# DeepGraphLearning/ULTRA

Measured on AMD Instinct MI355X. Metric: triples scored/sec (all-tail ranking) on FB15k237, higher is better.
Workload: dtype f32

## Files before the change

ultra_amd/csrc/dense_order_layer.hip:

```cpp
#include <hip/hip_runtime.h>

#include <cstdint>
#include <cstdlib>
#include <string>

#ifndef ULTRA_DOL_ASM
#define ULTRA_DOL_ASM 0
#endif
#if ULTRA_DOL_ASM
#include ULTRA_DOL_ASM_HEADER
#endif
#include "plan.hpp"
#include "torch_math.hpp"

#pragma clang fp contract(off)

namespace ultra {

using f32x4 = float __attribute__((ext_vector_type(4)));

enum { DOL_LN = 1, DOL_RELU = 2, DOL_RESIDUAL = 4 };

struct DenseOrderParams {
    const uint4 *a_ex;
    const float *rel, *x, *bnd;
    const long long *bnd_rows;
    const float *weight, *bias, *ln_w, *ln_b;
    float *out;
    long long rel_so, rel_sr, x_so, x_sr, bnd_so, bnd_sr, out_so, out_sr;
    int n_out, n_in, n_rel, n_jc, n_rt16, has_bnd, flags;
    float eps;
};

constexpr int DOL_ROW_STRIDE = 68;

__device__ __forceinline__ float byte_of(uint32_t w, int q) { return (float)((w >> (8 * q)) & 0xffu); }

#ifdef ULTRA_DOL_VGPR_CAP
#define ULTRA_DOL_ATTR __attribute__((amdgpu_waves_per_eu(4, 4)))
#else
#define ULTRA_DOL_ATTR
#endif
template <int TILES, bool LEAN, int SUBS = 1>
__device__ __forceinline__ void dense_order_layer_impl(const DenseOrderParams &p) {
    __shared__ __attribute__((aligned(16))) float x_lds_all[SUBS * TILES * 16 * DOL_ROW_STRIDE];
    __shared__ __attribute__((aligned(16))) float agg_lds_all[SUBS * TILES * 16 * DOL_ROW_STRIDE];
    __shared__ float ln_mom_all[SUBS][TILES * 16][8][2];
    __shared__ float ln_stat_all[SUBS][TILES * 16][2];
    const int sub = SUBS > 1 ? __builtin_amdgcn_readfirstlane((int)threadIdx.x >> 8) : 0;
    float *x_lds = x_lds_all + sub * (TILES * 16 * DOL_ROW_STRIDE), *agg_lds = agg_lds_all + sub * (TILES * 16 * DOL_ROW_STRIDE);
    float(&ln_mom)[TILES * 16][8][2] = ln_mom_all[sub];
    float(&ln_stat)[TILES * 16][2] = ln_stat_all[sub];
    const int tid = threadIdx.x & 255, lane = tid & 63;
    const int wave = __builtin_amdgcn_readfirstlane(tid >> 6);
    const int i16 = lane & 15, kk = lane >> 4;
    const int n_wt = (p.n_rt16 + TILES * SUBS - 1) / (TILES * SUBS);
    const int rt_raw = (blockIdx.x % n_wt) * SUBS + sub, outer = blockIdx.x / n_wt;
    const bool quartet_live = rt_raw * TILES < p.n_rt16;
    const int rt = quartet_live ? rt_raw : (p.n_rt16 - 1) / TILES;
    const float *xo = p.x + (long long)outer * p.x_so;
    const int row0 = rt * 16 * TILES;
    const int c0 = 16 * wave;
    const bool tile1 = TILES > 1 && TILES * rt + 1 < p.n_rt16;

    const uint4 *ap[TILES];
#pragma unroll
    for (int t = 0; t < TILES; ++t) ap[t] = p.a_ex + (size_t)min(TILES * rt + t, p.n_rt16 - 1) * p.n_jc * 64;
    const char *xbase = reinterpret_cast<const char *>(xo);
    const uint32_t x_row_bytes = (uint32_t)p.x_sr * 4u;
    const uint32_t lane_bytes = (uint32_t)(c0 + i16) * 4u;
#if !ULTRA_DOL_ASM
    uint32_t voff[16], voff_last[LEAN ? 1 : 16];
#pragma unroll
    for (int q = 0; q < 16; ++q) {
        voff[q] = (uint32_t)q * x_row_bytes + lane_bytes;
        if (!LEAN) voff_last[q] = (uint32_t)min(16 * (p.n_jc - 1) + q, p.n_in - 1) * x_row_bytes + lane_bytes;
    }
    const uint32_t off_max = (uint32_t)(p.n_in - 1 - 16 * (p.n_jc - 1)) * x_row_bytes + lane_bytes;
    struct Stage {
        uint4 a[TILES];
        float x[16];
    };
    const auto fetch = [&](const int jc, Stage &st) {
        const bool last = jc >= p.n_jc - 1;
        const int jcc = last ? p.n_jc - 1 : jc;
#pragma unroll
        for (int t = 0; t < TILES; ++t) st.a[t] = ap[t][(size_t)jcc * 64 + lane];
        if (LEAN) {
            const char *sbase = xbase + (uint32_t)jcc * 16u * x_row_bytes;
            const uint32_t cap = last ? off_max : 0xffffffffu;
#pragma unroll
            for (int q = 0; q < 16; ++q) st.x[q] = *reinterpret_cast<const float *>(sbase + min(voff[q], cap));
        } else {
            const char *sbase = xbase + (last ? 0u : (uint32_t)jcc * 16u * x_row_bytes);
#pragma unroll
            for (int q = 0; q < 16; ++q) st.x[q] = *reinterpret_cast<const float *>(sbase + (last ? voff_last[q] : voff[q]));
        }
    };
    Stage st0, st1, st2;
    fetch(0, st0);
    fetch(1, st1);
    fetch(2, st2);
#endif
    const float relv = kk < p.n_rel ? p.rel[(long long)outer * p.rel_so + (long long)kk * p.rel_sr + c0 + i16] : 0.f;

    float4 xtile[TILES];
    float wfrag[32];
    const int f0 = 16 * wave + 4 * kk;
    float biasv[4], lnw[4], lnb[4];
    float bndv[TILES][4];
    const auto fetch_late_operands = [&]() {
#pragma unroll
        for (int t = 0; t < TILES; ++t) {
            const int row = min(row0 + 16 * t + (tid >> 4), p.n_out - 1);
            xtile[t] = *reinterpret_cast<const float4 *>(xo + (long long)row * p.x_sr + 4 * (tid & 15));
        }
#pragma unroll
        for (int s = 0; s < 32; ++s) wfrag[s] = p.weight[(16 * wave + i16) * 128 + 4 * s + kk];
#pragma unroll
        for (int r = 0; r < 4; ++r) {
            biasv[r] = p.bias ? p.bias[f0 + r] : 0.f;
            lnw[r] = (p.flags & DOL_LN) ? p.ln_w[f0 + r] : 1.f;
            lnb[r] = (p.flags & DOL_LN) ? p.ln_b[f0 + r] : 0.f;
        }
#pragma unroll
        for (int t = 0; t < TILES; ++t)
#pragma unroll
            for (int r = 0; r < 4; ++r) bndv[t][r] = 0.f;
        if (p.has_bnd) {
            const long long bnd_row = p.bnd_rows ? p.bnd_rows[outer] : -1;
#pragma unroll
            for (int t = 0; t < TILES; ++t)
#pragma unroll
                for (int r = 0; r < 4; ++r) {
                    const int row = row0 + 16 * t + 4 * kk + r;
                    if (row < p.n_out && (bnd_row < 0 || bnd_row == row))
                        bndv[t][r] = p.bnd[(long long)outer * p.bnd_so + (long long)row * p.bnd_sr + c0 + i16];
                }
        }
    };
    if (!LEAN) fetch_late_operands();

    f32x4 acc[TILES];
#pragma unroll
    for (int t = 0; t < TILES; ++t)
#pragma unroll
        for (int r = 0; r < 4; ++r) acc[t][r] = 0.f;
#if ULTRA_DOL_ASM
    static_assert(TILES == 1, "the assembly chain of the measurement build walks one tile");
    dense_order_chain_asm(acc[0], p.n_jc, p.n_in, (uint32_t)lane * 16u, ap[0], xbase, lane_bytes, x_row_bytes, relv, (uint32_t)tid * 128u);
#else
    const auto chain = [&](const Stage &cur, const int jc) {
        const uint32_t m = jc < p.n_jc ? 0xffffffffu : 0u;
        uint32_t aw[TILES][4];
#pragma unroll
        for (int t = 0; t < TILES; ++t) {
            aw[t][0] = cur.a[t].x & m, aw[t][1] = cur.a[t].y & m, aw[t][2] = cur.a[t].z & m, aw[t][3] = cur.a[t].w & m;
        }
#pragma unroll
        for (int q = 0; q < 16; ++q) {
            const float b = relv * cur.x[q];
#pragma unroll
            for (int t = 0; t < TILES; ++t)
                acc[t] = __builtin_amdgcn_mfma_f32_16x16x4f32(byte_of(aw[t][q >> 2], q & 3), b, acc[t], 0, 0, 0);
        }
    };
    for (int jc = 0; jc < p.n_jc; jc += 3) {
        chain(st0, jc);
        fetch(jc + 3, st0);
        chain(st1, jc + 1);
        fetch(jc + 4, st1);
        chain(st2, jc + 2);
        fetch(jc + 5, st2);
    }
#endif

    if (LEAN) fetch_late_operands();

#pragma unroll
    for (int t = 0; t < TILES; ++t) {
#pragma unroll
        for (int r = 0; r < 4; ++r) {
            float v = acc[t][r];
            if (p.has_bnd) v += bndv[t][r];
            agg_lds[(16 * t + 4 * kk + r) * DOL_ROW_STRIDE + c0 + i16] = v;
        }
        *reinterpret_cast<float4 *>(x_lds + (16 * t + (tid >> 4)) * DOL_ROW_STRIDE + 4 * (tid & 15)) = xtile[t];
    }
    __syncthreads();

    f32x4 d[TILES];
#pragma unroll
    for (int t = 0; t < TILES; ++t) {
#pragma unroll
        for (int r = 0; r < 4; ++r) d[t][r] = 0.f;
#pragma unroll
        for (int s = 0; s < 16; ++s)
            d[t] = __builtin_amdgcn_mfma_f32_16x16x4f32(wfrag[s], x_lds[(16 * t + i16) * DOL_ROW_STRIDE + 4 * s + kk], d[t], 0, 0, 0);
#pragma unroll
        for (int s = 0; s < 16; ++s)
            d[t] = __builtin_amdgcn_mfma_f32_16x16x4f32(wfrag[16 + s], agg_lds[(16 * t + i16) * DOL_ROW_STRIDE + 4 * s + kk], d[t], 0, 0, 0);
    }
    float y[TILES][4];
#pragma unroll
    for (int t = 0; t < TILES; ++t)
#pragma unroll
        for (int r = 0; r < 4; ++r) y[t][r] = d[t][r] + biasv[r];
    if (p.flags & DOL_LN) {
        __syncthreads();
#pragma unroll
        for (int t = 0; t < TILES; ++t)
#pragma unroll
            for (int r = 0; r < 4; ++r) agg_lds[(16 * t + i16) * DOL_ROW_STRIDE + f0 + r] = y[t][r];
        __syncthreads();
        if (tid < 128 * TILES) {
            const int row = tid >> 3, i = tid & 7;
            float xv[8];
#pragma unroll
            for (int j = 0; j < 8; ++j) xv[j] = agg_lds[row * DOL_ROW_STRIDE + 8 * j + i];
            const Moments w = welford8(xv);
            ln_mom[row][i][0] = w.m1;
            ln_mom[row][i][1] = w.m2;
        }
        __syncthreads();
        if (tid < 16 * TILES) {
            Moments all[8];
#pragma unroll
            for (int i = 0; i < 8; ++i) all[i] = Moments{ln_mom[tid][i][0], ln_mom[tid][i][1]};
            float mean, rstd;
            merge8(all, p.eps, mean, rstd);
            ln_stat[tid][0] = mean;
            ln_stat[tid][1] = rstd;
        }
        __syncthreads();
#pragma unroll
        for (int t = 0; t < TILES; ++t) {
            const float mean = ln_stat[16 * t + i16][0], rstd = ln_stat[16 * t + i16][1];
#pragma unroll
            for (int r = 0; r < 4; ++r) y[t][r] = ln_apply(y[t][r], mean, rstd, lnw[r], lnb[r]);
        }
    }
#pragma unroll
    for (int t = 0; t < TILES; ++t) {
        if (p.flags & DOL_RELU) {
#pragma unroll
            for (int r = 0; r < 4; ++r) y[t][r] = fmaxf(y[t][r], 0.f);
        }
        if (p.flags & DOL_RESIDUAL) {
#pragma unroll
            for (int r = 0; r < 4; ++r) y[t][r] += x_lds[(16 * t + i16) * DOL_ROW_STRIDE + f0 + r];
        }
        const int row = row0 + 16 * t + i16;
        if (row < p.n_out && (t == 0 || tile1) && quartet_live)
            *reinterpret_cast<float4 *>(p.out + (long long)outer * p.out_so + (long long)row * p.out_sr + f0) =
                make_float4(y[t][0], y[t][1], y[t][2], y[t][3]);
    }
}

template <int TILES>
__global__ void __launch_bounds__(256) ULTRA_DOL_ATTR dense_order_layer_kernel(const DenseOrderParams p) {
    dense_order_layer_impl<TILES, false>(p);
}

__global__ void __launch_bounds__(256) __attribute__((amdgpu_waves_per_eu(4, 4))) dense_order_layer_lean_kernel(const DenseOrderParams p) {
    dense_order_layer_impl<1, true>(p);
}

__global__ void __launch_bounds__(1024) dense_order_layer_packed_kernel(const DenseOrderParams p) {
    dense_order_layer_impl<1, true, 4>(p);
}

static bool dol_ok16(const ultra_mat *m) {
    return (reinterpret_cast<uintptr_t>(m->ptr) & 15u) == 0 && m->stride_row % 4 == 0 && m->stride_outer % 4 == 0;
}

int launch_dense_order_layer(ultra_plan *p, const ultra_mat *rel, const ultra_mat *x, const ultra_mat *bnd, const int64_t *bnd_rows,
                             const void *weight, const void *bias, const void *ln_w, const void *ln_b, float eps, int flags,
                             const ultra_mat *out, hipStream_t stream, bool shared_chip) {
    if (!(p->flags & ULTRA_PLAN_DENSE) || p->a_ex.empty() || !p->d.a_ex) {
        set_error("ultra_nbf_dense_layer (reference order) needs a ULTRA_PLAN_DENSE plan of a graph with at most 4 relation types "
                  "whose parallel edges are sorted by type and never repeated");
        return ULTRA_ERR_UNSUPPORTED;
    }
    if (out->row_len != 64 || p->num_out != p->num_in) {
        set_error("ultra_nbf_dense_layer: hidden dim 64 on a square graph only");
        return ULTRA_ERR_UNSUPPORTED;
    }
    if (!dol_ok16(rel) || !dol_ok16(x) || !dol_ok16(out) || (bnd && !dol_ok16(bnd)) || (reinterpret_cast<uintptr_t>(weight) & 15u)) {
        set_error("ultra_nbf_dense_layer: operands must be 16-byte aligned with strides that are multiples of 4");
        return ULTRA_ERR_UNSUPPORTED;
    }
    if ((uint64_t)p->num_in * (uint64_t)x->stride_row * 4u >= (1ull << 32)) {
        set_error("ultra_nbf_dense_layer: an input slice (rows * stride_row) exceeds 4 GiB");
        return ULTRA_ERR_UNSUPPORTED;
    }
    DenseOrderParams dp;
    dp.a_ex = reinterpret_cast<const uint4 *>(p->d.a_ex);
    dp.rel = static_cast<const float *>(rel->ptr);
    dp.x = static_cast<const float *>(x->ptr);
    dp.bnd = bnd ? static_cast<const float *>(bnd->ptr) : nullptr;
    dp.bnd_rows = bnd ? reinterpret_cast<const long long *>(bnd_rows) : nullptr;
    dp.weight = static_cast<const float *>(weight);
    dp.bias = static_cast<const float *>(bias);
    dp.ln_w = static_cast<const float *>(ln_w);
    dp.ln_b = static_cast<const float *>(ln_b);
    dp.out = static_cast<float *>(out->ptr);
    dp.rel_so = rel->stride_outer, dp.rel_sr = rel->stride_row;
    dp.x_so = x->stride_outer, dp.x_sr = x->stride_row;
    dp.bnd_so = bnd ? bnd->stride_outer : 0, dp.bnd_sr = (bnd && !bnd_rows) ? bnd->stride_row : 0;
    dp.out_so = out->stride_outer, dp.out_sr = out->stride_row;
    dp.n_out = (int)p->num_out, dp.n_in = (int)p->num_in, dp.n_rel = (int)p->num_rel;
    dp.n_jc = (int)((p->num_in + 15) / 16), dp.n_rt16 = (int)((p->num_out + 15) / 16);
    dp.has_bnd = bnd ? 1 : 0;
    dp.flags = flags;
    dp.eps = eps;
    const char *tiles_str = std::getenv("ULTRA_DOL_TILES");
    const int tiles_env = tiles_str ? std::atoi(tiles_str) : 0;
    const char *lean_str = std::getenv("ULTRA_DOL_LEAN");
    const int lean = (ULTRA_DOL_ASM || tiles_env == 2) ? 0 : (lean_str ? std::atoi(lean_str) : (shared_chip ? 2 : 0));
    const int tiles = (ULTRA_DOL_ASM || dp.n_rt16 < 2) ? 1 : (tiles_env == 2 ? 2 : 1);
    const long long blocks = (long long)((dp.n_rt16 + tiles - 1) / tiles) * out->n_outer;
    if (tiles == 2) {
#if !ULTRA_DOL_ASM
        hipLaunchKernelGGL(dense_order_layer_kernel<2>, dim3((unsigned)blocks), dim3(256), 0, stream, dp);
#endif
    } else if (lean == 2 && dp.n_rt16 >= 4) {
#if !ULTRA_DOL_ASM
        const long long packed = (long long)((dp.n_rt16 + 3) / 4) * out->n_outer;
        hipLaunchKernelGGL(dense_order_layer_packed_kernel, dim3((unsigned)packed), dim3(1024), 0, stream, dp);
#endif
    } else if (lean) {
#if !ULTRA_DOL_ASM
        hipLaunchKernelGGL(dense_order_layer_lean_kernel, dim3((unsigned)blocks), dim3(256), 0, stream, dp);
#endif
    } else {
        hipLaunchKernelGGL(dense_order_layer_kernel<1>, dim3((unsigned)blocks), dim3(256), 0, stream, dp);
    }
    hipError_t e = hipGetLastError();
    if (e != hipSuccess) {
        set_error(std::string("dense_order_layer_kernel launch: ") + hipGetErrorString(e));
        return ULTRA_ERR_HIP;
    }
    return ULTRA_OK;
}

}
```

Baseline: 207.2 million.

## Add four-tile dense order layer with LDS-transposed x loads as shared-chip default

Adds a TILES=4 variant of the dense order layer kernel. Each block now computes four 16-row output tiles, so every x chunk fetched from memory is reused across four adjacency tiles. The x fetch becomes a single float4 per lane that is transposed through a small per-wave LDS buffer, and MFMAs are issued in groups separated by sched_barrier fences. On shared-chip runs with no env overrides this variant becomes the default in place of the packed lean kernel, trading occupancy (one wave per EU) and more registers for fewer x loads per output row.

Result: faster. 212.0 million (median of 6 runs) (+2.3%).

```diff
diff --git a/ultra_amd/csrc/dense_order_layer.hip b/ultra_amd/csrc/dense_order_layer.hip
--- a/ultra_amd/csrc/dense_order_layer.hip
+++ b/ultra_amd/csrc/dense_order_layer.hip
@@ -32,6 +32,8 @@
     float eps;
 };
 
+constexpr int DOL_GROUP = 4;
+constexpr int DOL_FENCE = 0x94;
 constexpr int DOL_ROW_STRIDE = 68;
 
 __device__ __forceinline__ float byte_of(uint32_t w, int q) { return (float)((w >> (8 * q)) & 0xffu); }
@@ -59,9 +61,13 @@
     const bool quartet_live = rt_raw * TILES < p.n_rt16;
     const int rt = quartet_live ? rt_raw : (p.n_rt16 - 1) / TILES;
     const float *xo = p.x + (long long)outer * p.x_so;
+    constexpr bool WIDE = TILES >= 4 && !ULTRA_DOL_ASM;
+    __shared__ __attribute__((aligned(16))) float xs_lds_all[WIDE ? 4 * 256 : 4];
     const int row0 = rt * 16 * TILES;
     const int c0 = 16 * wave;
-    const bool tile1 = TILES > 1 && TILES * rt + 1 < p.n_rt16;
+    bool tile_live[TILES];
+#pragma unroll
+    for (int t = 0; t < TILES; ++t) tile_live[t] = quartet_live && TILES * rt + t < p.n_rt16;
 
     const uint4 *ap[TILES];
 #pragma unroll
@@ -80,12 +86,20 @@
     struct Stage {
         uint4 a[TILES];
         float x[16];
+        float4 xw;
     };
+    float *xs_lds = xs_lds_all + (WIDE ? wave * 256 : 0);
+    const uint32_t wide_lane_bytes = (uint32_t)(c0 + 4 * (lane & 3)) * 4u;
     const auto fetch = [&](const int jc, Stage &st) {
         const bool last = jc >= p.n_jc - 1;
         const int jcc = last ? p.n_jc - 1 : jc;
 #pragma unroll
         for (int t = 0; t < TILES; ++t) st.a[t] = ap[t][(size_t)jcc * 64 + lane];
+        if (WIDE) {
+            const uint32_t row = (uint32_t)min(16 * jcc + (lane >> 2), p.n_in - 1);
+            st.xw = *reinterpret_cast<const float4 *>(xbase + row * x_row_bytes + wide_lane_bytes);
+            return;
+        }
         if (LEAN) {
             const char *sbase = xbase + (uint32_t)jcc * 16u * x_row_bytes;
             const uint32_t cap = last ? off_max : 0xffffffffu;
@@ -101,6 +115,12 @@
     fetch(0, st0);
     fetch(1, st1);
     fetch(2, st2);
+    const auto transpose = [&](Stage &st) {
+        if (!WIDE) return;
+        *reinterpret_cast<float4 *>(xs_lds + 4 * lane) = st.xw;
+#pragma unroll
+        for (int q = 0; q < 16; ++q) st.x[q] = xs_lds[16 * q + i16];
+    };
 #endif
     const float relv = kk < p.n_rel ? p.rel[(long long)outer * p.rel_so + (long long)kk * p.rel_sr + c0 + i16] : 0.f;
 
@@ -151,11 +171,30 @@
     dense_order_chain_asm(acc[0], p.n_jc, p.n_in, (uint32_t)lane * 16u, ap[0], xbase, lane_bytes, x_row_bytes, relv, (uint32_t)tid * 128u);
 #else
     const auto chain = [&](const Stage &cur, const int jc) {
-        const uint32_t m = jc < p.n_jc ? 0xffffffffu : 0u;
         uint32_t aw[TILES][4];
 #pragma unroll
         for (int t = 0; t < TILES; ++t) {
+            const uint32_t m = (jc < p.n_jc && (TILES == 1 || tile_live[t])) ? 0xffffffffu : 0u;
             aw[t][0] = cur.a[t].x & m, aw[t][1] = cur.a[t].y & m, aw[t][2] = cur.a[t].z & m, aw[t][3] = cur.a[t].w & m;
+        }
+        if (TILES >= 4) {
+#pragma unroll
+            for (int q0 = 0; q0 < 16; q0 += DOL_GROUP) {
+                float b[DOL_GROUP], af[DOL_GROUP][TILES];
+#pragma unroll
+                for (int g = 0; g < DOL_GROUP; ++g) {
+                    b[g] = relv * cur.x[q0 + g];
+#pragma unroll
+                    for (int t = 0; t < TILES; ++t) af[g][t] = byte_of(aw[t][(q0 + g) >> 2], (q0 + g) & 3);
+                }
+                __builtin_amdgcn_sched_barrier(DOL_FENCE);
+#pragma unroll
+                for (int g = 0; g < DOL_GROUP; ++g)
+#pragma unroll
+                    for (int t = 0; t < TILES; ++t) acc[t] = __builtin_amdgcn_mfma_f32_16x16x4f32(af[g][t], b[g], acc[t], 0, 0, 0);
+                __builtin_amdgcn_sched_barrier(DOL_FENCE);
+            }
+            return;
         }
 #pragma unroll
         for (int q = 0; q < 16; ++q) {
@@ -165,11 +204,15 @@
                 acc[t] = __builtin_amdgcn_mfma_f32_16x16x4f32(byte_of(aw[t][q >> 2], q & 3), b, acc[t], 0, 0, 0);
         }
     };
+    transpose(st0);
     for (int jc = 0; jc < p.n_jc; jc += 3) {
+        transpose(st1);
         chain(st0, jc);
         fetch(jc + 3, st0);
+        transpose(st2);
         chain(st1, jc + 1);
         fetch(jc + 4, st1);
+        transpose(st0);
         chain(st2, jc + 2);
         fetch(jc + 5, st2);
     }
@@ -213,14 +256,18 @@
 #pragma unroll
             for (int r = 0; r < 4; ++r) agg_lds[(16 * t + i16) * DOL_ROW_STRIDE + f0 + r] = y[t][r];
         __syncthreads();
-        if (tid < 128 * TILES) {
-            const int row = tid >> 3, i = tid & 7;
-            float xv[8];
-#pragma unroll
-            for (int j = 0; j < 8; ++j) xv[j] = agg_lds[row * DOL_ROW_STRIDE + 8 * j + i];
-            const Moments w = welford8(xv);
-            ln_mom[row][i][0] = w.m1;
-            ln_mom[row][i][1] = w.m2;
+#pragma unroll
+        for (int base = 0; base < 128 * TILES; base += 256) {
+            const int slot = base + tid;
+            if (slot < 128 * TILES) {
+                const int row = slot >> 3, i = slot & 7;
+                float xv[8];
+#pragma unroll
+                for (int j = 0; j < 8; ++j) xv[j] = agg_lds[row * DOL_ROW_STRIDE + 8 * j + i];
+                const Moments w = welford8(xv);
+                ln_mom[row][i][0] = w.m1;
+                ln_mom[row][i][1] = w.m2;
+            }
         }
         __syncthreads();
         if (tid < 16 * TILES) {
@@ -251,7 +298,7 @@
             for (int r = 0; r < 4; ++r) y[t][r] += x_lds[(16 * t + i16) * DOL_ROW_STRIDE + f0 + r];
         }
         const int row = row0 + 16 * t + i16;
-        if (row < p.n_out && (t == 0 || tile1) && quartet_live)
+        if (row < p.n_out && tile_live[t])
             *reinterpret_cast<float4 *>(p.out + (long long)outer * p.out_so + (long long)row * p.out_sr + f0) =
                 make_float4(y[t][0], y[t][1], y[t][2], y[t][3]);
     }
@@ -262,6 +309,13 @@
     dense_order_layer_impl<TILES, false>(p);
 }
 
+#if !ULTRA_DOL_ASM
+template <>
+__global__ void __launch_bounds__(256) __attribute__((amdgpu_waves_per_eu(1, 1))) dense_order_layer_kernel<4>(const DenseOrderParams p) {
+    dense_order_layer_impl<4, false>(p);
+}
+#endif
+
 __global__ void __launch_bounds__(256) __attribute__((amdgpu_waves_per_eu(4, 4))) dense_order_layer_lean_kernel(const DenseOrderParams p) {
     dense_order_layer_impl<1, true>(p);
 }
@@ -269,6 +323,8 @@
 __global__ void __launch_bounds__(1024) dense_order_layer_packed_kernel(const DenseOrderParams p) {
     dense_order_layer_impl<1, true, 4>(p);
 }
+
+constexpr bool DOL_SHARED_DEFAULT_TILES4 = true;
 
 static bool dol_ok16(const ultra_mat *m) {
     return (reinterpret_cast<uintptr_t>(m->ptr) & 15u) == 0 && m->stride_row % 4 == 0 && m->stride_outer % 4 == 0;
@@ -317,10 +373,19 @@
     const char *tiles_str = std::getenv("ULTRA_DOL_TILES");
     const int tiles_env = tiles_str ? std::atoi(tiles_str) : 0;
     const char *lean_str = std::getenv("ULTRA_DOL_LEAN");
-    const int lean = (ULTRA_DOL_ASM || tiles_env == 2) ? 0 : (lean_str ? std::atoi(lean_str) : (shared_chip ? 2 : 0));
-    const int tiles = (ULTRA_DOL_ASM || dp.n_rt16 < 2) ? 1 : (tiles_env == 2 ? 2 : 1);
+    int tiles = 1;
+    if (!ULTRA_DOL_ASM) {
+        if (tiles_env == 4 && dp.n_rt16 >= 4) tiles = 4;
+        else if (tiles_env == 2 && dp.n_rt16 >= 2) tiles = 2;
+        else if (DOL_SHARED_DEFAULT_TILES4 && !tiles_str && !lean_str && shared_chip && dp.n_rt16 >= 4) tiles = 4;
+    }
+    const int lean = (ULTRA_DOL_ASM || tiles > 1 || tiles_env == 2) ? 0 : (lean_str ? std::atoi(lean_str) : (shared_chip ? 2 : 0));
     const long long blocks = (long long)((dp.n_rt16 + tiles - 1) / tiles) * out->n_outer;
-    if (tiles == 2) {
+    if (tiles == 4) {
+#if !ULTRA_DOL_ASM
+        hipLaunchKernelGGL(dense_order_layer_kernel<4>, dim3((unsigned)blocks), dim3(256), 0, stream, dp);
+#endif
+    } else if (tiles == 2) {
 #if !ULTRA_DOL_ASM
         hipLaunchKernelGGL(dense_order_layer_kernel<2>, dim3((unsigned)blocks), dim3(256), 0, stream, dp);
 #endif
```
